# zhoubin-me/agent0

Hardware: AMD Instinct MI355X
Metric: env-frames/sec (learner FPS: transitions collected and saved to replay per second with the learner running, pre-frameskip) (higher is better)
Workload: dtype f32

## Files before the change

agent0_amd/csrc/conv1_wgrad.hip:

```cpp
#include "a0_internal.h"
#include "store_policy.h"
#include "update_tail.h"
typedef a0_st_wt a0_c1w_store;

#include <cstdint>

typedef __bf16 a0w_bf16x8 __attribute__((ext_vector_type(8)));
typedef uint32_t a0w_u32x4 __attribute__((ext_vector_type(4)));
typedef float a0w_acc4 __attribute__((ext_vector_type(4)));

constexpr int A0W_THREADS = 512;
constexpr int A0W_XP_ROW = 24, A0W_XP_PLANE = 21 * 24;
constexpr int A0W_XP_ELEMS = 64 * A0W_XP_PLANE;
constexpr int A0W_T_PITCH = 488, A0W_T_TERM = 32 * A0W_T_PITCH;
constexpr int A0W_GROUPS = 60;
constexpr int A0W_STEPS = 15;

struct a0_c1w_args {
    const uint8_t* frames; const int* slot; long long sample_stride; int chan_off;
    const float* d1;
    float* slabs;
    int B;
    a0_tail_prep prep;
};

A0_D uint32_t a0w_trunc(float f) { return __float_as_uint(f) >> 16; }
A0_D float a0w_up(uint32_t h) { return __uint_as_float(h << 16); }

__global__ __launch_bounds__(A0W_THREADS) void a0_conv1_wgrad_fused_kernel(a0_c1w_args P) {
    extern __shared__ __attribute__((aligned(16))) unsigned char smem[];
    uint16_t* Xp = (uint16_t*)smem;
    uint16_t* T = Xp + A0W_XP_ELEMS;
    const int tid = threadIdx.x, lane = tid & 63;
    const int wave = __builtin_amdgcn_readfirstlane(tid >> 6);
    const int q = lane >> 4, r16 = lane & 15;
    for (int i = tid; i < (A0W_XP_ELEMS + 3 * A0W_T_TERM) / 2; i += A0W_THREADS) ((uint32_t*)smem)[i] = 0u;
    int bbase[2], bshift[2];
#pragma unroll
    for (int t = 0; t < 2; ++t) {
        const int k = (2 * wave + t) * 16 + r16;
        const int c = k >> 6, kh = (k >> 3) & 7, kw = k & 7;
        const int plane = (c * 4 + (kh & 3)) * 4 + (kw & 3);
        bbase[t] = plane * A0W_XP_PLANE + (kh >> 2) * A0W_XP_ROW;
        bshift[t] = 2 * (kw >> 2);
    }
    a0w_acc4 acc[2][2];
#pragma unroll
    for (int i = 0; i < 2; ++i)
#pragma unroll
        for (int t = 0; t < 2; ++t) acc[i][t] = a0w_acc4{0.f, 0.f, 0.f, 0.f};
    float bsum = 0.f;
    __syncthreads();
    constexpr int NDW = 4 * 84 * 21, TR = (NDW + A0W_THREADS - 1) / A0W_THREADS;
    constexpr int GT = (A0W_GROUPS + A0W_THREADS / 32 - 1) / (A0W_THREADS / 32);
    uint32_t w[TR];
    float v[GT][8];
    auto load_raw = [&](int b) {
        const long long s = P.slot ? (long long)P.slot[b] : (long long)b;
        const uint32_t* src = (const uint32_t*)(P.frames + s * P.sample_stride + P.chan_off);
#pragma unroll
        for (int j = 0; j < TR; ++j) { const int i = tid + j * A0W_THREADS; w[j] = src[i < NDW ? i : NDW - 1]; }
        const float* g = P.d1 + (long long)b * 400 * 32 + (tid & 31);
#pragma unroll
        for (int t = 0; t < GT; ++t) {
            int G = (tid >> 5) + t * (A0W_THREADS / 32);
            G = G < A0W_GROUPS ? G : A0W_GROUPS - 1;
            const int oh = G / 3, ow0 = 8 * (G - 3 * oh);
#pragma unroll
            for (int j = 0; j < 8; ++j) { const int m = oh * 20 + ow0 + j; v[t][j] = g[(m < 400 ? m : 399) * 32]; }
        }
    };
    load_raw(blockIdx.x);
    for (int b = blockIdx.x; b < P.B; b += gridDim.x) {
#pragma unroll
        for (int j = 0; j < TR; ++j) {
            int i = tid + j * A0W_THREADS;
            i = i < NDW ? i : NDW - 1;
            const int c = i / (84 * 21), rem = i - c * (84 * 21), y = rem / 21, xc = rem - y * 21;
            uint16_t* d = Xp + ((c * 4 + (y & 3)) * 4) * A0W_XP_PLANE + (y >> 2) * A0W_XP_ROW + xc;
            d[0 * A0W_XP_PLANE] = (uint16_t)(__float_as_uint((float)(w[j] & 0xffu)) >> 16);
            d[1 * A0W_XP_PLANE] = (uint16_t)(__float_as_uint((float)((w[j] >> 8) & 0xffu)) >> 16);
            d[2 * A0W_XP_PLANE] = (uint16_t)(__float_as_uint((float)((w[j] >> 16) & 0xffu)) >> 16);
            d[3 * A0W_XP_PLANE] = (uint16_t)(__float_as_uint((float)(w[j] >> 24)) >> 16);
        }
        {
            const int n = tid & 31;
#pragma unroll
            for (int t = 0; t < GT; ++t) {
                const int G = (tid >> 5) + t * (A0W_THREADS / 32);
                if (G < A0W_GROUPS) {
                    const int oh = G / 3, ow0 = 8 * (G - 3 * oh);
                    uint32_t t0[4], t1[4], t2[4];
#pragma unroll
                    for (int j = 0; j < 8; j += 2) {
                        uint32_t h[2], m[2], l[2];
#pragma unroll
                        for (int e = 0; e < 2; ++e) {
                            const float x = (ow0 + j + e < 20) ? v[t][j + e] : 0.f;
                            bsum += x;
                            h[e] = a0w_trunc(x);
                            const float r1 = x - a0w_up(h[e]);
                            m[e] = a0w_trunc(r1);
                            l[e] = a0w_trunc(r1 - a0w_up(m[e]));
                        }
                        t0[j >> 1] = h[0] | (h[1] << 16); t1[j >> 1] = m[0] | (m[1] << 16); t2[j >> 1] = l[0] | (l[1] << 16);
                    }
                    uint16_t* d = T + n * A0W_T_PITCH + 8 * G;
                    *(uint4*)(d) = uint4{t0[0], t0[1], t0[2], t0[3]};
                    *(uint4*)(d + A0W_T_TERM) = uint4{t1[0], t1[1], t1[2], t1[3]};
                    *(uint4*)(d + 2 * A0W_T_TERM) = uint4{t2[0], t2[1], t2[2], t2[3]};
                }
            }
        }
        __syncthreads();
        if (b + (int)gridDim.x < P.B) load_raw(b + gridDim.x);
        {
            const uint16_t* ap = T + r16 * A0W_T_PITCH + 8 * q;
            const uint16_t* bp0 = Xp + bbase[0] + 8 * q;
            const uint16_t* bp1 = Xp + bbase[1] + 8 * q;
#pragma unroll 3
            for (int st = 0; st < A0W_STEPS; ++st) {
                a0w_u32x4 a[2][3], bf[2];
#pragma unroll
                for (int i = 0; i < 2; ++i)
#pragma unroll
                    for (int s3 = 0; s3 < 3; ++s3) {
                        const uint4 x = *(const uint4*)(ap + s3 * A0W_T_TERM + i * 16 * A0W_T_PITCH + 32 * st);
                        a[i][s3] = a0w_u32x4{x.x, x.y, x.z, x.w};
                    }
#pragma unroll
                for (int t = 0; t < 2; ++t) {
                    const uint16_t* bp = (t == 0 ? bp0 : bp1) + 32 * st;
                    const uint4 lo = *(const uint4*)bp;
                    const uint32_t hi = *(const uint32_t*)(bp + 8);
                    const int sh = bshift[t];
                    bf[t] = a0w_u32x4{__builtin_amdgcn_alignbyte(lo.y, lo.x, sh), __builtin_amdgcn_alignbyte(lo.z, lo.y, sh),
                                      __builtin_amdgcn_alignbyte(lo.w, lo.z, sh), __builtin_amdgcn_alignbyte(hi, lo.w, sh)};
                }
#pragma unroll
                for (int s3 = 0; s3 < 3; ++s3)
#pragma unroll
                    for (int i = 0; i < 2; ++i)
#pragma unroll
                        for (int t = 0; t < 2; ++t)
                            acc[i][t] = __builtin_amdgcn_mfma_f32_16x16x32_bf16(__builtin_bit_cast(a0w_bf16x8, a[i][s3]), __builtin_bit_cast(a0w_bf16x8, bf[t]), acc[i][t], 0, 0, 0);
            }
        }
        __syncthreads();
    }
    float* out = P.slabs + (long long)blockIdx.x * (32 * 256 + 32);
#pragma unroll
    for (int i = 0; i < 2; ++i)
#pragma unroll
        for (int t = 0; t < 2; ++t) {
            const int k = (2 * wave + t) * 16 + r16;
#pragma unroll
            for (int r = 0; r < 4; ++r) a0_store4<a0_c1w_store>(&out[(i * 16 + 4 * q + r) * 256 + k], __float_as_uint(acc[i][t][r] / 255.0f));
        }
    float* red = (float*)smem;
    red[tid] = bsum;
    __syncthreads();
    if (tid < 32) {
        float s = 0.f;
#pragma unroll
        for (int j = 0; j < A0W_THREADS / 32; ++j) s += red[j * 32 + tid];
        out[32 * 256 + tid] = s;
    }
    if (P.prep.state != nullptr && blockIdx.x == 0 && tid == 0) a0_tail_prep_run(P.prep);
}

int a0_conv1_wgrad_fused_launch(const a0_frames_arg* f, int C, int H, int W, int B, const float* d1, float* slabs, const a0_tail_prep* prep, hipStream_t st) {
    if (C != 4 || H != 84 || W != 84 || B < 1 || (f->sample_stride & 3) || (f->chan_off & 3) || (((uintptr_t)f->frames) & 3)) return 0;
    a0_c1w_args P;
    P.frames = f->frames; P.slot = f->slot; P.sample_stride = f->sample_stride; P.chan_off = f->chan_off;
    P.d1 = d1; P.slabs = slabs; P.B = B;
    P.prep = prep ? *prep : a0_tail_prep{nullptr, nullptr, 0.0, 0.0, 0.0, 0};
    const int grid = B < 256 ? B : 256;
    const size_t lds = (size_t)(A0W_XP_ELEMS + 3 * A0W_T_TERM) * 2;
    static bool configured = false;
    if (!configured) {
        A0_HIP_THROW(hipFuncSetAttribute((const void*)a0_conv1_wgrad_fused_kernel, hipFuncAttributeMaxDynamicSharedMemorySize, (int)lds));
        configured = true;
    }
    hipLaunchKernelGGL(a0_conv1_wgrad_fused_kernel, dim3(grid), dim3(A0W_THREADS), lds, st, P);
    A0_HIP_THROW(hipGetLastError());
    return grid;
}
```

agent0_amd/csrc/encoder_fused.hip:

```cpp
#include "a0_internal.h"
#include "net_tables.h"
#include "operands.h"
#include "store_policy.h"
#include "update_tail.h"

#include <cstdlib>
#include <type_traits>

typedef float a0_acc4 __attribute__((ext_vector_type(4)));

struct a0_fused_args {
    const uint8_t* frames; const int* slot; long long sample_stride; int chan_off;
    const float *wt1, *wt2, *wt3;
    const float *wx2, *wx3;
    const float *b1, *b2, *b3;
    float *act1, *act2, *act3;
    int B;
    int C, H, W, H1, W1, H2, W2, H3, W3;
    int off_act1, off_act2, off_end;
    int rp1, rp2;
};

A0_HD void a0_fused_set_wt(a0_fused_args& P, const float* wt, int C) {
    const a0_wt_layout T{C};
// ... 381 lines not shown
        *(a0_f4*)(glb + (unsigned)(m * N + n0)) = a0_f4{v[0], v[1], v[2], v[3]};
    }
};

struct a0_live_all {
    static constexpr bool all = true;
    static constexpr int steps = 2;
    static constexpr bool live(int, int) { return true; }
};
template <int ORD, int N, int WN, int MBT, int R, int LR, class LIVE = a0_live_all, class AFX, class EPI, class Between>
A0_D void a0_conv_stage_x9k(const AFX& af, int M, a0_wring9<N, WN, R, A0_FUSED_WAVES / WN>& ring, const EPI& epi, float* xch0, float* xch1, Between&& between) {
    constexpr int WK = A0_FUSED_WAVES / WN, HB0 = (MBT + 1) / 2, HB1 = MBT / 2;
    static_assert(WK == 2 && N == 16 * WN && HB1 >= 1 && EPI::TR && LR >= 1 && LR <= 16, "tile shape");
    const int tid = threadIdx.x, lane = tid & 63;
    const int wave = __builtin_amdgcn_readfirstlane(tid >> 6);
    const int wn = wave % WN, wk = wave / WN;
    const int q = lane >> 4, r16 = lane & 15;
    const int MB = (M + 15) >> 4, NSTW = LIVE::all ? ring.nst : LIVE::steps / WK;
    static_assert(LIVE::all || (LIVE::steps % (WK * R)) == 0, "own k steps: a multiple of the ring depth");
    auto live = [](int blk, int j) { return j < LIVE::steps / WK && (LIVE::live(blk, WK * j) || LIVE::live(blk, WK * j + 1)); };
    int rows[MBT];
#pragma unroll
    for (int i = 0; i < MBT; ++i) {
        const int m = i * 16 + r16;
        rows[i] = af.row(m < M ? m : 0) + 8 * q;
    }
    a0_acc4 acc[MBT];
#pragma unroll
    for (int i = 0; i < MBT; ++i) acc[i] = a0_acc4{0.f, 0.f, 0.f, 0.f};
    uint4 a[2][HB0][3];
    auto fetch = [&](int slot, int h, int off, int j) {
#pragma unroll
        for (int i = 0; i < HB0; ++i)
            if (h * HB0 + i < MBT) {
                if constexpr (!LIVE::all) { if (!live(h * HB0 + i, j)) continue; }
#pragma unroll
                for (int t = 0; t < 3; ++t) a[slot][i][t] = *(const uint4*)(af.planes + rows[h * HB0 + i] + off + t * AFX::term);
            }
    };
    fetch(0, 0, af.step_off(wk), 0);
    __builtin_amdgcn_s_waitcnt(0x0F70);
    if constexpr (!LIVE::all) asm volatile("" : "+v"(ring.p));
#pragma unroll LIVE::all ? 1 : LIVE::steps / (WK * R)
    for (int tb = 0; tb < NSTW; tb += R) {
#pragma unroll
        for (int u = 0; u < R; ++u) {
            const int st = wk + WK * (tb + u);
            const int off = af.step_off(st), offn = af.step_off(tb + u + 1 < NSTW ? st + WK : st);
#pragma unroll
            for (int h = 0; h < 2; ++h) {
                if (h == 0) fetch(1, 1, off, tb + u);
                else fetch(0, 0, offn, tb + u + 1);
                __builtin_amdgcn_sched_barrier(0);
#pragma unroll
                for (int ta = 0; ta < 3; ++ta)
#pragma unroll
                    for (int tw = 0; tw < 3; ++tw)
#pragma unroll
                        for (int i = 0; i < HB0; ++i) {
                            if (ta + tw > ORD || h * HB0 + i >= MBT) continue;
                            if constexpr (!LIVE::all) { if (!live(h * HB0 + i, tb + u)) continue; }
                            const a0_u32x4 av = {a[h][i][ta].x, a[h][i][ta].y, a[h][i][ta].z, a[h][i][ta].w};
                            const a0_u32x4 bv = {ring.v[u][0][tw].x, ring.v[u][0][tw].y, ring.v[u][0][tw].z, ring.v[u][0][tw].w};
                            acc[h * HB0 + i] = __builtin_amdgcn_mfma_f32_16x16x32_bf16(__builtin_bit_cast(a0_bf16x8, bv), __builtin_bit_cast(a0_bf16x8, av), acc[h * HB0 + i], 0, 0, 0);
                        }
                __builtin_amdgcn_sched_barrier(0);
            }
            ring.fill(u);
            __builtin_amdgcn_sched_barrier(0);
        }
    }
    between();
    a0_acc4* x0 = (a0_acc4*)xch0;
    a0_acc4* x1 = (a0_acc4*)xch1;
    constexpr int P1 = (HB1 - 1) * 64 + 4 * LR;
    const int last = q * LR + r16;
    const int n0 = wn * 16 + 4 * q;
    float pe[EPI::PER_ELEM ? HB0 : 1][4];
    auto send = [&](auto mine) {
        constexpr int H = decltype(mine)::value;
        if constexpr (EPI::PER_ELEM) {
#pragma unroll
            for (int i = 0; i < (H == 0 ? HB0 : HB1); ++i) {
                const int m = (H * HB0 + i) * 16 + r16;
                const a0_f4 v = epi.pre_elem4(m < M ? m : M - 1, n0);
                pe[i][0] = v.x; pe[i][1] = v.y; pe[i][2] = v.z; pe[i][3] = v.w;
            }
        }
        if constexpr (H == 1) {
#pragma unroll
            for (int i = 0; i < HB0; ++i) x0[(wn * HB0 + i) * 64 + lane] = acc[i];
        } else {
#pragma unroll
            for (int i = 0; i < HB1; ++i) {
                if (i < HB1 - 1) x1[wn * P1 + i * 64 + lane] = acc[HB0 + i];
                else if (r16 < LR) x1[wn * P1 + (HB1 - 1) * 64 + last] = acc[HB0 + i];
            }
        }
    };
    auto recv = [&](auto mine) {
        constexpr int H = decltype(mine)::value;
#pragma unroll
        for (int i = 0; i < (H == 0 ? HB0 : HB1); ++i) {
            const int mb = H * HB0 + i;
            const int m = mb * 16 + r16;
            if constexpr (H == 0) acc[mb] += x0[(wn * HB0 + i) * 64 + lane];
            else {
                if (i < HB1 - 1) acc[mb] += x1[wn * P1 + i * 64 + lane];
                else if (r16 < LR) acc[mb] += x1[wn * P1 + (HB1 - 1) * 64 + last];
            }
            if (mb < MB && m < M) epi.emit_n4(m, n0, acc[mb], EPI::PER_ELEM ? pe[EPI::PER_ELEM ? i : 0] : nullptr);
        }
    };
    if (wk == 0) send(std::integral_constant<int, 0>{});
    else send(std::integral_constant<int, 1>{});
    __syncthreads();
    if (wk == 0) recv(std::integral_constant<int, 0>{});
    else recv(std::integral_constant<int, 1>{});
    __syncthreads();
}
constexpr int A0_P1X = 40, A0_P2X = 80;
constexpr int A0_RP1X = 20 * A0_P1X + 8;
constexpr int A0_RP2X = 9 * A0_P2X + 96;

constexpr int A0_R1 = 4, A0_R2 = 4, A0_R3 = 6;

template <int MBW1, int MBW2, int MBW3, int WC, bool X9, bool LOOP = false, int ORD = 4>
__global__ __launch_bounds__(A0_FUSED_THREADS) void a0_encoder_fused_kernel(a0_fused_args P);

constexpr int A0_X9_BIAS_OFF = 2 * 4 * 84 * 84 + 3 * 20 * A0_RP1X * 2;
constexpr int A0_RK2 = 2, A0_RK3 = 3;
constexpr int A0_X9_XCH0 = 3 * 9 * A0_RP2X * 2;
constexpr int A0_X9_XCH1 = A0_X9_BIAS_OFF + 160 * 4;
static_assert(A0_X9_XCH0 + 4 * 3 * 1024 <= 2 * 4 * 84 * 84, "conv2 exchange region 0 fits into the image");
constexpr int A0_X9_LDS_BYTES = A0_X9_XCH1 + 4 * (2 * 64 + 4) * 16;
static_assert(A0_X9_LDS_BYTES <= 160 * 1024, "LDS");
static_assert(A0_FUSED_WAVES == 8, "N-stationary stages: four waves along N, two along K");
typedef a0_wring9<64, 4, A0_RK2, 2> a0_ring2_t;
typedef a0_wring9<64, 4, A0_RK3, 2> a0_ring3_t;
template <int ORD, bool LOOP>
A0_D void a0_x9_conv23(const a0_fused_args& P, int b, unsigned char* smem, float* bias_lds, a0_wring1<A0_R1>& ring1, a0_ring2_t& ring2, a0_ring3_t& ring3) {
    const int obs_bytes = P.C * P.H * P.W;
    const int M2 = P.H2 * P.W2, M3 = P.H3 * P.W3;
    uint16_t* a1p = (uint16_t*)(smem + 2 * obs_bytes);
    constexpr int term1 = 20 * A0_RP1X, term2 = 9 * A0_RP2X;
    uint16_t* a2p = (uint16_t*)smem;
    typedef EpiFwdX<9, A0_P2X, A0_RP2X, term2> E2X;
    const AF2X<term1> f2{a1p, A0_RP1X, P.W2, A0_P1X};
    const E2X e2{bias_lds + 32, a2p, P.act2 ? P.act2 + (long long)b * M2 * 64 : nullptr, 64};
    const AF3X<term2> f3{a2p, A0_RP2X, P.W3, A0_P2X};
    const EpiFwdT e3{bias_lds + 96, P.act3 + (long long)b * M3 * 64, 64};
    a0_conv_stage_x9k<ORD, 64, 4, 6, A0_RK2, 1>(f2, M2, ring2, e2, (float*)(smem + A0_X9_XCH0), (float*)(smem + A0_X9_XCH1), [&] { ring3.prologue(); });
    a0_conv_stage_x9k<ORD, 64, 4, 4, A0_RK3, 16>(f3, M3, ring3, e3, (float*)a1p, (float*)a1p + 4 * 2 * 256, [&] { if (LOOP) ring1.prologue(); });
}

A0_D void a0_bytes16_to_img(uint16_t* img, int idx16, const uint4& v) {
    const uint32_t w[4] = {v.x, v.y, v.z, v.w};
    uint32_t o[8];
#pragma unroll
    for (int k = 0; k < 4; ++k) {
        const uint32_t f0 = __float_as_uint((float)(w[k] & 0xffu)), f1 = __float_as_uint((float)((w[k] >> 8) & 0xffu));
        const uint32_t f2 = __float_as_uint((float)((w[k] >> 16) & 0xffu)), f3 = __float_as_uint((float)(w[k] >> 24));
        o[2 * k] = __builtin_amdgcn_perm(f1, f0, 0x07060302u);
        o[2 * k + 1] = __builtin_amdgcn_perm(f3, f2, 0x07060302u);
    }
    ((uint4*)img)[2 * idx16] = uint4{o[0], o[1], o[2], o[3]};
    ((uint4*)img)[2 * idx16 + 1] = uint4{o[4], o[5], o[6], o[7]};
}

template <int ORD, bool LOOP>
A0_D void a0_encoder_fused_x9_body(const a0_fused_args& P, int bid, int nblk) {
    extern __shared__ __attribute__((aligned(16))) unsigned char smem[];
    uint16_t* img = (uint16_t*)smem;
    const int obs_bytes = P.C * P.H * P.W;
    const int M1 = P.H1 * P.W1;
    uint16_t* a1p = (uint16_t*)(smem + 2 * obs_bytes);
    constexpr int term1 = 20 * A0_RP1X;
    typedef EpiFwdX<20, A0_P1X, A0_RP1X, term1> E1X;
    a0_wring1<A0_R1> ring1;
    a0_ring2_t ring2;
    a0_ring3_t ring3;
    ring1.init(P.wt1, P.C);
    ring2.init(P.wx2, 512);
    ring3.init(P.wx3, 576);
    ring1.prologue();
    constexpr int MBW1X = (25 + A0_WMG1 - 1) / A0_WMG1;
    a0_pre<32, 2, MBW1X, E1X> pre1;
    float* bias_lds = (float*)(smem + A0_X9_BIAS_OFF);
    if (threadIdx.x < 160) bias_lds[threadIdx.x] = threadIdx.x < 32 ? P.b1[threadIdx.x] : threadIdx.x < 96 ? P.b2[threadIdx.x - 32] : P.b3[threadIdx.x - 96];
    for (int b = bid; b < P.B; b += nblk) {
        const long long s = P.slot ? (long long)P.slot[b] : (long long)b;
        const uint4* src = (const uint4*)(P.frames + s * P.sample_stride + P.chan_off);
        constexpr int TRIPS = 4;
        const int n16 = obs_bytes >> 4;
        for (int i0 = threadIdx.x; i0 < n16; i0 += TRIPS * A0_FUSED_THREADS) {
            uint4 v[TRIPS];
#pragma unroll
            for (int j = 0; j < TRIPS; ++j) {
                const int i = i0 + j * A0_FUSED_THREADS;
                v[j] = src[i < n16 ? i : n16 - 1];
            }
#pragma unroll
            for (int j = 0; j < TRIPS; ++j) {
                const int i = i0 + j * A0_FUSED_THREADS;
                a0_bytes16_to_img(img, i < n16 ? i : n16 - 1, v[j]);
            }
        }
        __syncthreads();
        const E1X e1{bias_lds, a1p, P.act1 ? P.act1 + (long long)b * M1 * 32 : nullptr, 32};
        const int wmg1 = __builtin_amdgcn_readfirstlane(threadIdx.x >> 6) / 2;
        if (MBW1X > 1 && wmg1 + (MBW1X - 1) * A0_WMG1 >= ((M1 + 15) >> 4))
            a0_conv1_stage<(MBW1X > 1 ? MBW1X - 1 : 1), A0_R1, 84>(img, P.H * P.W, P.W, P.W1, M1, ring1, e1, pre1, [&] { ring2.prologue(); });
        else
            a0_conv1_stage<MBW1X, A0_R1, 84>(img, P.H * P.W, P.W, P.W1, M1, ring1, e1, pre1, [&] { ring2.prologue(); });
        a0_x9_conv23<ORD, LOOP>(P, b, smem, bias_lds, ring1, ring2, ring3);
        if constexpr (!LOOP) break;
    }
}

#include "actor_tail.h"
typedef a0_st_nt a0_step_row_store;
struct a0_step_enc_args { const float *wt, *b1, *b2, *b3; float* act3; };
template <int ORD>
__global__ __launch_bounds__(A0_FUSED_THREADS) void a0_actor_dist_step_enc_kernel(a0_dtenv_args Q, a0_step_enc_args N) {
    __shared__ int s_chase_cell;
    extern __shared__ __attribute__((aligned(16))) unsigned char smem[];
    unsigned long long v_wt = (unsigned long long)N.wt, v_b1 = (unsigned long long)N.b1, v_b2 = (unsigned long long)N.b2, v_b3 = (unsigned long long)N.b3,
                       v_a3 = (unsigned long long)N.act3, v_obs = (unsigned long long)Q.obs_out;
    A0_TO_VGPR(v_wt); A0_TO_VGPR(v_b1); A0_TO_VGPR(v_b2); A0_TO_VGPR(v_b3); A0_TO_VGPR(v_a3); A0_TO_VGPR(v_obs);
    int v_E = Q.E;
    A0_TO_VGPR(v_E);
    a0_actor_dist_tail_env_body(Q, (float*)smem, &s_chase_cell);
    __syncthreads();
    auto uni = [](unsigned long long v) {
        return ((unsigned long long)(unsigned)__builtin_amdgcn_readfirstlane((int)(v >> 32)) << 32) | (unsigned long long)(unsigned)__builtin_amdgcn_readfirstlane((int)(v & 0xffffffffull));
    };
    const float* wt = (const float*)uni(v_wt);
    a0_fused_args P;
    P.frames = (const uint8_t*)uni(v_obs); P.slot = nullptr; P.sample_stride = 4 * 84 * 84; P.chan_off = 0;
    a0_fused_set_wt(P, wt, 4);
    P.b1 = (const float*)uni(v_b1); P.b2 = (const float*)uni(v_b2); P.b3 = (const float*)uni(v_b3);
    P.act1 = nullptr; P.act2 = nullptr; P.act3 = (float*)uni(v_a3); P.B = __builtin_amdgcn_readfirstlane(v_E);
    P.C = 4; P.H = 84; P.W = 84; P.H1 = 20; P.W1 = 20; P.H2 = 9; P.W2 = 9; P.H3 = 7; P.W3 = 7;
    P.off_act1 = 0; P.off_act2 = 0; P.off_end = 0; P.rp1 = 0; P.rp2 = 0;
    a0_encoder_fused_x9_body<ORD, false>(P, (int)blockIdx.x, (int)gridDim.x);
}

template <int MBW, class EPI, class Mid, class Between>
A0_D void a0_conv1_stage_split(const uint16_t* img, a0_wring1<A0_R1>& ring, const EPI& epi, bool first_before_mid, Mid&& mid, Between&& between) {
    static_assert(A0_R1 == 4 && EPI::TR, "ring of four steps, transposed accumulators");
    constexpr int HW = 84 * 84, W = 84, W1 = 20, M = 400, MB = 25;
    const int tid = threadIdx.x, lane = tid & 63;
    const int wave = __builtin_amdgcn_readfirstlane(tid >> 6);
    const int wn = wave % 2, wmg = wave / 2;
    const int q = lane >> 4, r16 = lane & 15;
    int rows[MBW];
#pragma unroll
    for (int i = 0; i < MBW; ++i) {
        int m = (wmg + i * A0_WMG1) * 16 + r16;
        m = m < M ? m : 0;
        const int oh = m / W1, ow = m - oh * W1;
        rows[i] = (4 * oh + q) * W + 4 * ow;
    }
    a0_acc4 acc[MBW];
#pragma unroll
    for (int i = 0; i < MBW; ++i) acc[i] = a0_acc4{0.f, 0.f, 0.f, 0.f};
    uint2 a[2][MBW][2];
    auto fetch = [&](int slot, int off) {
#pragma unroll
        for (int i = 0; i < MBW; ++i) {
            a[slot][i][0] = *(const uint2*)(img + rows[i] + off);
            a[slot][i][1] = *(const uint2*)(img + rows[i] + off + 4);
        }
    };
    auto off_of = [&](int st) { return (st >> 1) * HW + (st & 1) * 4 * W; };
    auto step = [&](auto UC, int off_next) {
        constexpr int u = decltype(UC)::value;
        fetch((u + 1) & 1, off_next);
        __builtin_amdgcn_sched_barrier(0);
#pragma unroll
        for (int s3 = 0; s3 < 3; ++s3)
#pragma unroll
            for (int i = 0; i < MBW; ++i) {
                const a0_u32x4 av = {a[u & 1][i][0].x, a[u & 1][i][0].y, a[u & 1][i][1].x, a[u & 1][i][1].y};
                const a0_u32x4 bv = {ring.v[u][s3].x, ring.v[u][s3].y, ring.v[u][s3].z, ring.v[u][s3].w};
                acc[i] = __builtin_amdgcn_mfma_f32_16x16x32_bf16(__builtin_bit_cast(a0_bf16x8, bv), __builtin_bit_cast(a0_bf16x8, av), acc[i], 0, 0, 0);
            }
        __builtin_amdgcn_sched_barrier(0);
        ring.fill(u);
        __builtin_amdgcn_sched_barrier(0);
    };
    typedef std::integral_constant<int, 0> U0; typedef std::integral_constant<int, 1> U1; typedef std::integral_constant<int, 2> U2; typedef std::integral_constant<int, 3> U3;
    auto steps05 = [&] {
        fetch(0, off_of(0));
        __builtin_amdgcn_s_waitcnt(0x0F70);
        step(U0{}, off_of(1)); step(U1{}, off_of(2)); step(U2{}, off_of(3)); step(U3{}, off_of(4));
        step(U0{}, off_of(5)); step(U1{}, off_of(5));
    };
    if (first_before_mid) steps05();
    mid();
    if (!first_before_mid) steps05();
    fetch(0, off_of(6));
    __builtin_amdgcn_s_waitcnt(0x0F70);
    step(U2{}, off_of(7)); step(U3{}, off_of(7));
    between();
#pragma unroll
    for (int i = 0; i < MBW; ++i) {
        const int mb = wmg + i * A0_WMG1;
        if (mb < MB) {
            const int m = mb * 16 + r16;
            if (m < M) epi.emit_n4(m, wn * 16 + 4 * q, acc[i], nullptr);
        }
    }
    __syncthreads();
}

struct TailScalar {
    typedef a0_qenv_args Args;
    static A0_D void run(const a0_qenv_args& Q, uint32_t e, uint32_t g, long long steps, unsigned long long off_a, unsigned long long off_u, float eps, long long slot, const a0_u4& x,
                         bool chase, int lane, float* w2s , float* raw, int* s_chase_cell_p) {
// ... 615 lines not shown
```

agent0_amd/csrc/operands.h:

```cpp
#pragma once
#include "a0_defs.h"
#include "store_policy.h"

enum { A0_KC = 0, A0_XC = 1 };

struct a0_frames_src {
    const uint8_t* frames;
    const int* slot;
    a0_geom g;
    int chan_off;
    const a0_i4* ktab;
    int aligned4;
};

A0_HD uint32_t a0_u8x4_load(const uint8_t* p, int aligned4) {
    if (aligned4) return *(const uint32_t*)p;
    return (uint32_t)p[0] | ((uint32_t)p[1] << 8) | ((uint32_t)p[2] << 16) | ((uint32_t)p[3] << 24);
}

A0_HD float a0_div255(float x) {
    const float r = 1.0f / 255.0f;
    const float q0 = x * r;
#if defined(__HIPCC__)
    const float e = __builtin_fmaf(-q0, 255.0f, x);
    return __builtin_fmaf(e, r, q0);
#else
    const float e = __builtin_fmaf(-q0, 255.0f, x);
    return __builtin_fmaf(e, r, q0);
#endif
}

A0_HD a0_f4 a0_u8x4_to_f4(uint32_t w, bool valid) {
    if (!valid) w = 0;
    a0_f4 v;
    v.x = a0_div255((float)(w & 255u));
    v.y = a0_div255((float)((w >> 8) & 255u));
    v.z = a0_div255((float)((w >> 16) & 255u));
    v.w = a0_div255((float)(w >> 24));
    return v;
}

A0_HD const uint8_t* a0_frames_row(const a0_frames_src& P, int m) {
    int b = a0_udiv(m, P.g.HWout, P.g.hw_magic);
    int rem = m - b * P.g.HWout;
    int oh = a0_udiv(rem, P.g.Wout, P.g.w_magic);
    int ow = rem - oh * P.g.Wout;
    long long s = P.slot ? (long long)P.slot[b] : (long long)b;
    return P.frames + s * P.g.sample_stride + P.chan_off + (long long)(oh * P.g.stride) * P.g.Win + ow * P.g.stride;
}

struct OpFramesKC {
    static constexpr int MODE = A0_KC;
    typedef a0_frames_src Params;
    struct Row { const uint8_t* p; bool ok; };
    struct KInfo { int off; bool ok; };
    A0_HD static Row row(const Params& P, int m, int M) {
        Row r; r.ok = m < M; r.p = a0_frames_row(P, r.ok ? m : 0); return r;
    }
    A0_HD static KInfo kinfo(const Params& P, int k, int Kend) {
        KInfo ki; ki.ok = k < Kend; ki.off = P.ktab[ki.ok ? (k >> 2) : 0].x; return ki;
    }
    typedef uint32_t Raw;
    A0_HD static Raw load(const Params& P, const Row& r, const KInfo& ki, bool& ok) {
        ok = r.ok && ki.ok;
        return a0_u8x4_load(r.p + ki.off, P.aligned4);
    }
    A0_HD static a0_f4 finish(Raw w, bool ok) { return a0_u8x4_to_f4(w, ok); }
};

struct OpFramesXC {
    static constexpr int MODE = A0_XC;
    typedef a0_frames_src Params;
    struct XInfo { int off; bool ok; };
    A0_HD static XInfo xinfo(const Params& P, int x, int X) {
        XInfo xi; xi.ok = x < X; xi.off = P.ktab[xi.ok ? (x >> 2) : 0].x; return xi;
    }
    typedef uint32_t Raw;
    A0_HD static Raw load(const Params& P, int m, int Mend, const XInfo& xi, bool& ok) {
        ok = xi.ok && m < Mend;
        return a0_u8x4_load(a0_frames_row(P, ok ? m : 0) + xi.off, P.aligned4);
    }
    A0_HD static a0_f4 finish(Raw w, bool ok) { return a0_u8x4_to_f4(w, ok); }
};

struct a0_act_src {
    const float* x;
    a0_geom g;
    const a0_i4* ktab;
};

struct a0_act_row { long long base; int h0, w0; bool ok; };

A0_HD a0_act_row a0_act_rowdesc(const a0_act_src& P, int m, bool ok) {
    a0_act_row r;
    if (!ok) m = 0;
    int b = a0_udiv(m, P.g.HWout, P.g.hw_magic);
    int rem = m - b * P.g.HWout;
    int oh = a0_udiv(rem, P.g.Wout, P.g.w_magic);
    int ow = rem - oh * P.g.Wout;
    r.h0 = oh * P.g.stride - P.g.pad;
    r.w0 = ow * P.g.stride - P.g.pad;
    r.base = (long long)b * P.g.sample_stride + ((long long)r.h0 * P.g.Win + r.w0) * P.g.C;
    r.ok = ok;
    return r;
}

A0_HD a0_f4 a0_act_fetch(const a0_act_src& P, const a0_act_row& r, const a0_i4& t, bool kok, bool& ok) {
    const int h = r.h0 + t.y, w = r.w0 + t.z;
    ok = r.ok && kok && (unsigned)h < (unsigned)P.g.Hin && (unsigned)w < (unsigned)P.g.Win;
    return *(const a0_f4*)(P.x + (ok ? r.base + t.x : 0));
}

A0_HD a0_f4 a0_f4_select(a0_f4 v, bool ok) { if (!ok) v = a0_zero4(); return v; }

struct OpActKC {
    static constexpr int MODE = A0_KC;
    typedef a0_act_src Params;
    typedef a0_act_row Row;
    struct KInfo { a0_i4 t; bool ok; };
    A0_HD static Row row(const Params& P, int m, int M) { return a0_act_rowdesc(P, m, m < M); }
    A0_HD static KInfo kinfo(const Params& P, int k, int Kend) {
        KInfo ki; ki.ok = k < Kend; ki.t = P.ktab[ki.ok ? (k >> 2) : 0]; return ki;
    }
    typedef a0_f4 Raw;
    A0_HD static Raw load(const Params& P, const Row& r, const KInfo& ki, bool& ok) { return a0_act_fetch(P, r, ki.t, ki.ok, ok); }
    A0_HD static a0_f4 finish(Raw v, bool ok) { return a0_f4_select(v, ok); }
};

struct OpActXC {
    static constexpr int MODE = A0_XC;
    typedef a0_act_src Params;
    struct XInfo { a0_i4 t; bool ok; };
    A0_HD static XInfo xinfo(const Params& P, int x, int X) {
        XInfo xi; xi.ok = x < X; xi.t = P.ktab[xi.ok ? (x >> 2) : 0]; return xi;
    }
    typedef a0_f4 Raw;
    A0_HD static Raw load(const Params& P, int m, int Mend, const XInfo& xi, bool& ok) {
        return a0_act_fetch(P, a0_act_rowdesc(P, m, m < Mend), xi.t, xi.ok, ok);
    }
    A0_HD static a0_f4 finish(Raw v, bool ok) { return a0_f4_select(v, ok); }
};

struct a0_mat_src { const float* x; int ld; };

struct OpMatKC {
    static constexpr int MODE = A0_KC;
    typedef a0_mat_src Params;
    struct Row { const float* p; bool ok; };
    struct KInfo { int k; bool ok; };
    A0_HD static Row row(const Params& P, int r, int R) { Row o; o.ok = r < R; o.p = P.x + (o.ok ? (long long)r * P.ld : 0); return o; }
    A0_HD static KInfo kinfo(const Params&, int k, int Kend) { KInfo ki; ki.ok = k < Kend; ki.k = ki.ok ? k : 0; return ki; }
    typedef a0_f4 Raw;
    A0_HD static Raw load(const Params&, const Row& r, const KInfo& ki, bool& ok) {
        ok = r.ok && ki.ok;
        return *(const a0_f4*)(r.p + ki.k);
    }
    A0_HD static a0_f4 finish(Raw v, bool ok) { return a0_f4_select(v, ok); }
};

struct OpMatXC {
    static constexpr int MODE = A0_XC;
    typedef a0_mat_src Params;
    struct XInfo { int x; bool ok; };
    A0_HD static XInfo xinfo(const Params&, int x, int X) { XInfo xi; xi.ok = x < X; xi.x = xi.ok ? x : 0; return xi; }
    typedef a0_f4 Raw;
    A0_HD static Raw load(const Params& P, int k, int Kend, const XInfo& xi, bool& ok) {
        ok = xi.ok && k < Kend;
        return *(const a0_f4*)(P.x + (ok ? (long long)k * P.ld : 0) + xi.x);
    }
    A0_HD static a0_f4 finish(Raw v, bool ok) { return a0_f4_select(v, ok); }
};

struct a0_wtab_src { const float* w; const int* wtab; };

struct OpWtabXC {
    static constexpr int MODE = A0_XC;
    typedef a0_wtab_src Params;
    struct XInfo { int x; bool ok; };
    A0_HD static XInfo xinfo(const Params&, int x, int X) { XInfo xi; xi.ok = x < X; xi.x = xi.ok ? x : 0; return xi; }
    typedef a0_f4 Raw;
    A0_HD static Raw load(const Params& P, int k, int Kend, const XInfo& xi, bool& ok) {
        ok = xi.ok && k < Kend;
        return *(const a0_f4*)(P.w + P.wtab[ok ? k : 0] + xi.x);
    }
    A0_HD static a0_f4 finish(Raw v, bool ok) { return a0_f4_select(v, ok); }
};

struct EpiBiasAct {
    static constexpr bool ROWSUM_A = false;
    struct Params { float* out; const float* bias; int ld; int relu; };
    A0_HD static void store(const Params& P, int x, int y, float v, int) {
        v += P.bias[y];
        if (P.relu) v = (v < 0.f) ? 0.f : v;
// ... 59 lines not shown
```

Measured before the change: 2.567 million.

## Restructure conv1 wgrad LDS layout using transposed LDS reads and plain image

Rewrites the conv1 weight-gradient kernel to stage the frame as a row-major bf16 image (reusing the shared bytes-to-image helper) and the d1 gradient in a swizzled 64-byte-row layout. MFMA fragments are then fetched with ds_read_tr16_b64 transposed LDS reads, replacing the stride-4 phase-plane layout and the alignbyte shuffles. Global loads become 16-byte vector loads, the per-iteration LDS zeroing shrinks to padding only, and the bias sum is rebuilt from the fragments already loaded. In exchange it relies on the MI355X-specific transpose-read instruction and tighter padding and swizzle invariants, which carry correctness risk.

```diff
diff --git a/agent0_amd/csrc/conv1_wgrad.hip b/agent0_amd/csrc/conv1_wgrad.hip
--- a/agent0_amd/csrc/conv1_wgrad.hip
+++ b/agent0_amd/csrc/conv1_wgrad.hip
@@ -1,4 +1,5 @@
 #include "a0_internal.h"
+#include "operands.h"
 #include "store_policy.h"
 #include "update_tail.h"
 typedef a0_st_wt a0_c1w_store;
@@ -6,15 +7,23 @@
 #include <cstdint>
 
 typedef __bf16 a0w_bf16x8 __attribute__((ext_vector_type(8)));
+typedef short a0w_s16x4 __attribute__((ext_vector_type(4)));
+typedef uint32_t a0w_u32x2 __attribute__((ext_vector_type(2)));
 typedef uint32_t a0w_u32x4 __attribute__((ext_vector_type(4)));
 typedef float a0w_acc4 __attribute__((ext_vector_type(4)));
+typedef uint32_t a0w_u32x4_a4 __attribute__((ext_vector_type(4), aligned(4)));
+typedef float a0w_f32x4_a4 __attribute__((ext_vector_type(4), aligned(4)));
 
 constexpr int A0W_THREADS = 512;
-constexpr int A0W_XP_ROW = 24, A0W_XP_PLANE = 21 * 24;
-constexpr int A0W_XP_ELEMS = 64 * A0W_XP_PLANE;
-constexpr int A0W_T_PITCH = 488, A0W_T_TERM = 32 * A0W_T_PITCH;
-constexpr int A0W_GROUPS = 60;
+constexpr int A0W_ROW = 64;
+constexpr int A0W_T_TERM = 20 * 24 * A0W_ROW;
+constexpr int A0W_IMG_PITCH = 84 * 2, A0W_IMG_CHAN = 84 * A0W_IMG_PITCH;
+constexpr int A0W_IMG_BYTES = 4 * A0W_IMG_CHAN;
+constexpr int A0W_IMG_TAIL = 32;
+constexpr int A0W_LDS_BYTES = 3 * A0W_T_TERM + A0W_IMG_BYTES + A0W_IMG_TAIL;
 constexpr int A0W_STEPS = 15;
+static_assert((3 * A0W_T_TERM) % 256 == 0 && A0W_IMG_BYTES % 16 == 0, "the image starts on a bank row; 16-byte stores reach its tail");
+static_assert(3 * A0W_IMG_CHAN + (4 * 19 + 7) * A0W_IMG_PITCH + 2 * (4 * 23 + 4) + 8 == A0W_IMG_BYTES + A0W_IMG_TAIL, "the last transposed read ends with the tail");
 
 struct a0_c1w_args {
     const uint8_t* frames; const int* slot; long long sample_stride; int chan_off;
@@ -24,25 +33,78 @@
     a0_tail_prep prep;
 };
 
-A0_D uint32_t a0w_trunc(float f) { return __float_as_uint(f) >> 16; }
-A0_D float a0w_up(uint32_t h) { return __uint_as_float(h << 16); }
+A0_D void a0w_split4(const a0_f4& v, a0w_u32x2& hi, a0w_u32x2& mid, a0w_u32x2& lo) {
+    const float x[4] = {v.x, v.y, v.z, v.w};
+    uint32_t h[4], m[4], l[4];
+#pragma unroll
+    for (int e = 0; e < 4; ++e) {
+        h[e] = __float_as_uint(x[e]);
+        const float r1 = x[e] - __uint_as_float(h[e] & 0xffff0000u);
+        m[e] = __float_as_uint(r1);
+        l[e] = __float_as_uint(r1 - __uint_as_float(m[e] & 0xffff0000u));
+    }
+    hi.x = __builtin_amdgcn_perm(h[1], h[0], 0x07060302u);  hi.y = __builtin_amdgcn_perm(h[3], h[2], 0x07060302u);
+    mid.x = __builtin_amdgcn_perm(m[1], m[0], 0x07060302u); mid.y = __builtin_amdgcn_perm(m[3], m[2], 0x07060302u);
+    lo.x = __builtin_amdgcn_perm(l[1], l[0], 0x07060302u);  lo.y = __builtin_amdgcn_perm(l[3], l[2], 0x07060302u);
+}
+
+A0_D a0w_u32x4 a0w_frag(const unsigned char* p0, const unsigned char* p1) {
+    typedef __attribute__((address_space(3))) a0w_s16x4 lds_s16x4;
+    const a0w_s16x4 k03 = __builtin_amdgcn_ds_read_tr16_b64_v4i16((lds_s16x4*)p0);
+    const a0w_s16x4 k47 = __builtin_amdgcn_ds_read_tr16_b64_v4i16((lds_s16x4*)p1);
+    const a0w_u32x2 a = __builtin_bit_cast(a0w_u32x2, k03), b = __builtin_bit_cast(a0w_u32x2, k47);
+    return a0w_u32x4{a.x, a.y, b.x, b.y};
+}
 
 __global__ __launch_bounds__(A0W_THREADS) void a0_conv1_wgrad_fused_kernel(a0_c1w_args P) {
     extern __shared__ __attribute__((aligned(16))) unsigned char smem[];
-    uint16_t* Xp = (uint16_t*)smem;
-    uint16_t* T = Xp + A0W_XP_ELEMS;
+    unsigned char* const T = smem;
+    unsigned char* const img = smem + 3 * A0W_T_TERM;
     const int tid = threadIdx.x, lane = tid & 63;
     const int wave = __builtin_amdgcn_readfirstlane(tid >> 6);
     const int q = lane >> 4, r16 = lane & 15;
-    for (int i = tid; i < (A0W_XP_ELEMS + 3 * A0W_T_TERM) / 2; i += A0W_THREADS) ((uint32_t*)smem)[i] = 0u;
-    int bbase[2], bshift[2];
+    constexpr int N16 = 4 * 84 * 84 / 16, TR = (N16 + A0W_THREADS - 1) / A0W_THREADS;
+    constexpr int NF4 = 400 * 8, TD = (NF4 + A0W_THREADS - 1) / A0W_THREADS;
+    uint4 w[TR];
+    a0_f4 v[TD];
+    auto load_raw = [&](int b) {
+        const long long s = P.slot ? (long long)P.slot[b] : (long long)b;
+        const uint8_t* src = P.frames + s * P.sample_stride + P.chan_off;
+        const float* g = P.d1 + (long long)b * 400 * 32;
+#pragma unroll
+        for (int j = 0; j < TR; ++j) {
+            const int i = tid + j * A0W_THREADS;
+            const a0w_u32x4_a4 x = ((const a0w_u32x4_a4*)src)[i < N16 ? i : N16 - 1];
+            w[j] = uint4{x[0], x[1], x[2], x[3]};
+        }
+#pragma unroll
+        for (int j = 0; j < TD; ++j) {
+            const int i = tid + j * A0W_THREADS;
+            const a0w_f32x4_a4 x = ((const a0w_f32x4_a4*)g)[i < NF4 ? i : NF4 - 1];
+            v[j].x = x[0]; v[j].y = x[1]; v[j].z = x[2]; v[j].w = x[3];
+        }
+    };
+    load_raw(blockIdx.x);
+    for (int i = tid; i < 3 * 20 * 16 + A0W_IMG_TAIL / 16; i += A0W_THREADS) {
+        const int term = i / 320, rem = i - term * 320;
+        unsigned char* d = i < 960 ? T + term * A0W_T_TERM + ((rem >> 4) * 24 + 20) * A0W_ROW + (rem & 15) * 16 : img + A0W_IMG_BYTES + (i - 960) * 16;
+        *(uint4*)d = uint4{0u, 0u, 0u, 0u};
+    }
+    int doff[TD];
+#pragma unroll
+    for (int j = 0; j < TD; ++j) {
+        int i = tid + j * A0W_THREADS;
+        i = i < NF4 ? i : NF4 - 1;
+        const int pos = i >> 3, m = pos + 4 * (pos / 20);
+        doff[j] = m * A0W_ROW + ((8 * (i & 7)) ^ (32 * ((m >> 3) & 1)));
+    }
+    const int fr = r16 >> 2, fp = r16 & 3;
+    const int aoff = (8 * q + fr) * A0W_ROW + ((8 * fp) ^ (32 * (q & 1)));
+    int bbase[2];
 #pragma unroll
     for (int t = 0; t < 2; ++t) {
-        const int k = (2 * wave + t) * 16 + r16;
-        const int c = k >> 6, kh = (k >> 3) & 7, kw = k & 7;
-        const int plane = (c * 4 + (kh & 3)) * 4 + (kw & 3);
-        bbase[t] = plane * A0W_XP_PLANE + (kh >> 2) * A0W_XP_ROW;
-        bshift[t] = 2 * (kw >> 2);
+        const int tb = 2 * wave + t, c = tb >> 2, kh0 = 2 * (tb & 3);
+        bbase[t] = c * A0W_IMG_CHAN + (kh0 + (fp >> 1)) * A0W_IMG_PITCH + 8 * (fp & 1) + 8 * fr;
     }
     a0w_acc4 acc[2][2];
 #pragma unroll
@@ -50,100 +112,49 @@
 #pragma unroll
         for (int t = 0; t < 2; ++t) acc[i][t] = a0w_acc4{0.f, 0.f, 0.f, 0.f};
     float bsum = 0.f;
-    __syncthreads();
-    constexpr int NDW = 4 * 84 * 21, TR = (NDW + A0W_THREADS - 1) / A0W_THREADS;
-    constexpr int GT = (A0W_GROUPS + A0W_THREADS / 32 - 1) / (A0W_THREADS / 32);
-    uint32_t w[TR];
-    float v[GT][8];
-    auto load_raw = [&](int b) {
-        const long long s = P.slot ? (long long)P.slot[b] : (long long)b;
-        const uint32_t* src = (const uint32_t*)(P.frames + s * P.sample_stride + P.chan_off);
-#pragma unroll
-        for (int j = 0; j < TR; ++j) { const int i = tid + j * A0W_THREADS; w[j] = src[i < NDW ? i : NDW - 1]; }
-        const float* g = P.d1 + (long long)b * 400 * 32 + (tid & 31);
-#pragma unroll
-        for (int t = 0; t < GT; ++t) {
-            int G = (tid >> 5) + t * (A0W_THREADS / 32);
-            G = G < A0W_GROUPS ? G : A0W_GROUPS - 1;
-            const int oh = G / 3, ow0 = 8 * (G - 3 * oh);
-#pragma unroll
-            for (int j = 0; j < 8; ++j) { const int m = oh * 20 + ow0 + j; v[t][j] = g[(m < 400 ? m : 399) * 32]; }
-        }
-    };
-    load_raw(blockIdx.x);
     for (int b = blockIdx.x; b < P.B; b += gridDim.x) {
 #pragma unroll
-        for (int j = 0; j < TR; ++j) {
-            int i = tid + j * A0W_THREADS;
-            i = i < NDW ? i : NDW - 1;
-            const int c = i / (84 * 21), rem = i - c * (84 * 21), y = rem / 21, xc = rem - y * 21;
-            uint16_t* d = Xp + ((c * 4 + (y & 3)) * 4) * A0W_XP_PLANE + (y >> 2) * A0W_XP_ROW + xc;
-            d[0 * A0W_XP_PLANE] = (uint16_t)(__float_as_uint((float)(w[j] & 0xffu)) >> 16);
-            d[1 * A0W_XP_PLANE] = (uint16_t)(__float_as_uint((float)((w[j] >> 8) & 0xffu)) >> 16);
-            d[2 * A0W_XP_PLANE] = (uint16_t)(__float_as_uint((float)((w[j] >> 16) & 0xffu)) >> 16);
-            d[3 * A0W_XP_PLANE] = (uint16_t)(__float_as_uint((float)(w[j] >> 24)) >> 16);
-        }
-        {
-            const int n = tid & 31;
+        for (int j = 0; j < TR; ++j) { const int i = tid + j * A0W_THREADS; a0_bytes16_to_img((uint16_t*)img, i < N16 ? i : N16 - 1, w[j]); }
 #pragma unroll
-            for (int t = 0; t < GT; ++t) {
-                const int G = (tid >> 5) + t * (A0W_THREADS / 32);
-                if (G < A0W_GROUPS) {
-                    const int oh = G / 3, ow0 = 8 * (G - 3 * oh);
-                    uint32_t t0[4], t1[4], t2[4];
-#pragma unroll
-                    for (int j = 0; j < 8; j += 2) {
-                        uint32_t h[2], m[2], l[2];
-#pragma unroll
-                        for (int e = 0; e < 2; ++e) {
-                            const float x = (ow0 + j + e < 20) ? v[t][j + e] : 0.f;
-                            bsum += x;
-                            h[e] = a0w_trunc(x);
-                            const float r1 = x - a0w_up(h[e]);
-                            m[e] = a0w_trunc(r1);
-                            l[e] = a0w_trunc(r1 - a0w_up(m[e]));
-                        }
-                        t0[j >> 1] = h[0] | (h[1] << 16); t1[j >> 1] = m[0] | (m[1] << 16); t2[j >> 1] = l[0] | (l[1] << 16);
-                    }
-                    uint16_t* d = T + n * A0W_T_PITCH + 8 * G;
-                    *(uint4*)(d) = uint4{t0[0], t0[1], t0[2], t0[3]};
-                    *(uint4*)(d + A0W_T_TERM) = uint4{t1[0], t1[1], t1[2], t1[3]};
-                    *(uint4*)(d + 2 * A0W_T_TERM) = uint4{t2[0], t2[1], t2[2], t2[3]};
-                }
-            }
+        for (int j = 0; j < TD; ++j) {
+            a0w_u32x2 hi, mid, lo;
+            a0w_split4(v[j], hi, mid, lo);
+            unsigned char* d = T + doff[j];
+            *(a0w_u32x2*)d = hi; *(a0w_u32x2*)(d + A0W_T_TERM) = mid; *(a0w_u32x2*)(d + 2 * A0W_T_TERM) = lo;
         }
         __syncthreads();
         if (b + (int)gridDim.x < P.B) load_raw(b + gridDim.x);
-        {
-            const uint16_t* ap = T + r16 * A0W_T_PITCH + 8 * q;
-            const uint16_t* bp0 = Xp + bbase[0] + 8 * q;
-            const uint16_t* bp1 = Xp + bbase[1] + 8 * q;
 #pragma unroll 3
-            for (int st = 0; st < A0W_STEPS; ++st) {
-                a0w_u32x4 a[2][3], bf[2];
+        for (int st = 0; st < A0W_STEPS; ++st) {
+            a0w_u32x4 a[2][3], bf[2];
+#pragma unroll
+            for (int i = 0; i < 2; ++i)
+#pragma unroll
+                for (int s3 = 0; s3 < 3; ++s3) {
+                    const unsigned char* x = T + (aoff ^ (32 * i)) + s3 * A0W_T_TERM + 32 * A0W_ROW * st;
+                    a[i][s3] = a0w_frag(x, x + 4 * A0W_ROW);
+                }
+            {
+                const unsigned G = 4u * st + q, oh = G / 3u;
+                const unsigned char* bp = img + oh * (4 * A0W_IMG_PITCH) + (G - 3u * oh) * 64;
+#pragma unroll
+                for (int t = 0; t < 2; ++t) bf[t] = a0w_frag(bp + bbase[t], bp + bbase[t] + 32);
+            }
+#pragma unroll
+            for (int s3 = 0; s3 < 3; ++s3)
 #pragma unroll
                 for (int i = 0; i < 2; ++i)
 #pragma unroll
-                    for (int s3 = 0; s3 < 3; ++s3) {
-                        const uint4 x = *(const uint4*)(ap + s3 * A0W_T_TERM + i * 16 * A0W_T_PITCH + 32 * st);
-                        a[i][s3] = a0w_u32x4{x.x, x.y, x.z, x.w};
-                    }
+                    for (int t = 0; t < 2; ++t)
+                        acc[i][t] = __builtin_amdgcn_mfma_f32_16x16x32_bf16(__builtin_bit_cast(a0w_bf16x8, a[i][s3]), __builtin_bit_cast(a0w_bf16x8, bf[t]), acc[i][t], 0, 0, 0);
+            if (((st ^ wave) & 3) == 0) {
+                const bool up = wave >= 4;
 #pragma unroll
-                for (int t = 0; t < 2; ++t) {
-                    const uint16_t* bp = (t == 0 ? bp0 : bp1) + 32 * st;
-                    const uint4 lo = *(const uint4*)bp;
-                    const uint32_t hi = *(const uint32_t*)(bp + 8);
-                    const int sh = bshift[t];
-                    bf[t] = a0w_u32x4{__builtin_amdgcn_alignbyte(lo.y, lo.x, sh), __builtin_amdgcn_alignbyte(lo.z, lo.y, sh),
-                                      __builtin_amdgcn_alignbyte(lo.w, lo.z, sh), __builtin_amdgcn_alignbyte(hi, lo.w, sh)};
+                for (int e = 0; e < 4; ++e) {
+                    const uint32_t h = up ? a[1][0][e] : a[0][0][e], m = up ? a[1][1][e] : a[0][1][e], l = up ? a[1][2][e] : a[0][2][e];
+                    bsum += (__uint_as_float(h << 16) + __uint_as_float(m << 16)) + __uint_as_float(l << 16);
+                    bsum += (__uint_as_float(h & 0xffff0000u) + __uint_as_float(m & 0xffff0000u)) + __uint_as_float(l & 0xffff0000u);
                 }
-#pragma unroll
-                for (int s3 = 0; s3 < 3; ++s3)
-#pragma unroll
-                    for (int i = 0; i < 2; ++i)
-#pragma unroll
-                        for (int t = 0; t < 2; ++t)
-                            acc[i][t] = __builtin_amdgcn_mfma_f32_16x16x32_bf16(__builtin_bit_cast(a0w_bf16x8, a[i][s3]), __builtin_bit_cast(a0w_bf16x8, bf[t]), acc[i][t], 0, 0, 0);
             }
         }
         __syncthreads();
@@ -158,7 +169,7 @@
             for (int r = 0; r < 4; ++r) a0_store4<a0_c1w_store>(&out[(i * 16 + 4 * q + r) * 256 + k], __float_as_uint(acc[i][t][r] / 255.0f));
         }
     float* red = (float*)smem;
-    red[tid] = bsum;
+    red[(4 * (wave & 3) + q) * 32 + 16 * (wave >> 2) + r16] = bsum;
     __syncthreads();
     if (tid < 32) {
         float s = 0.f;
@@ -176,7 +187,7 @@
     P.d1 = d1; P.slabs = slabs; P.B = B;
     P.prep = prep ? *prep : a0_tail_prep{nullptr, nullptr, 0.0, 0.0, 0.0, 0};
     const int grid = B < 256 ? B : 256;
-    const size_t lds = (size_t)(A0W_XP_ELEMS + 3 * A0W_T_TERM) * 2;
+    const size_t lds = (size_t)A0W_LDS_BYTES;
     static bool configured = false;
     if (!configured) {
         A0_HIP_THROW(hipFuncSetAttribute((const void*)a0_conv1_wgrad_fused_kernel, hipFuncAttributeMaxDynamicSharedMemorySize, (int)lds));
diff --git a/agent0_amd/csrc/encoder_fused.hip b/agent0_amd/csrc/encoder_fused.hip
--- a/agent0_amd/csrc/encoder_fused.hip
+++ b/agent0_amd/csrc/encoder_fused.hip
@@ -557,20 +557,6 @@
     const EpiFwdT e3{bias_lds + 96, P.act3 + (long long)b * M3 * 64, 64};
     a0_conv_stage_x9k<ORD, 64, 4, 6, A0_RK2, 1>(f2, M2, ring2, e2, (float*)(smem + A0_X9_XCH0), (float*)(smem + A0_X9_XCH1), [&] { ring3.prologue(); });
     a0_conv_stage_x9k<ORD, 64, 4, 4, A0_RK3, 16>(f3, M3, ring3, e3, (float*)a1p, (float*)a1p + 4 * 2 * 256, [&] { if (LOOP) ring1.prologue(); });
-}
-
-A0_D void a0_bytes16_to_img(uint16_t* img, int idx16, const uint4& v) {
-    const uint32_t w[4] = {v.x, v.y, v.z, v.w};
-    uint32_t o[8];
-#pragma unroll
-    for (int k = 0; k < 4; ++k) {
-        const uint32_t f0 = __float_as_uint((float)(w[k] & 0xffu)), f1 = __float_as_uint((float)((w[k] >> 8) & 0xffu));
-        const uint32_t f2 = __float_as_uint((float)((w[k] >> 16) & 0xffu)), f3 = __float_as_uint((float)(w[k] >> 24));
-        o[2 * k] = __builtin_amdgcn_perm(f1, f0, 0x07060302u);
-        o[2 * k + 1] = __builtin_amdgcn_perm(f3, f2, 0x07060302u);
-    }
-    ((uint4*)img)[2 * idx16] = uint4{o[0], o[1], o[2], o[3]};
-    ((uint4*)img)[2 * idx16 + 1] = uint4{o[4], o[5], o[6], o[7]};
 }
 
 template <int ORD, bool LOOP>
diff --git a/agent0_amd/csrc/operands.h b/agent0_amd/csrc/operands.h
--- a/agent0_amd/csrc/operands.h
+++ b/agent0_amd/csrc/operands.h
@@ -39,6 +39,22 @@
     v.w = a0_div255((float)(w >> 24));
     return v;
 }
+
+#if defined(__HIPCC__)
+A0_D void a0_bytes16_to_img(uint16_t* img, int idx16, const uint4& v) {
+    const uint32_t w[4] = {v.x, v.y, v.z, v.w};
+    uint32_t o[8];
+#pragma unroll
+    for (int k = 0; k < 4; ++k) {
+        const uint32_t f0 = __float_as_uint((float)(w[k] & 0xffu)), f1 = __float_as_uint((float)((w[k] >> 8) & 0xffu));
+        const uint32_t f2 = __float_as_uint((float)((w[k] >> 16) & 0xffu)), f3 = __float_as_uint((float)(w[k] >> 24));
+        o[2 * k] = __builtin_amdgcn_perm(f1, f0, 0x07060302u);
+        o[2 * k + 1] = __builtin_amdgcn_perm(f3, f2, 0x07060302u);
+    }
+    ((uint4*)img)[2 * idx16] = uint4{o[0], o[1], o[2], o[3]};
+    ((uint4*)img)[2 * idx16 + 1] = uint4{o[4], o[5], o[6], o[7]};
+}
+#endif
 
 A0_HD const uint8_t* a0_frames_row(const a0_frames_src& P, int m) {
     int b = a0_udiv(m, P.g.HWout, P.g.hw_magic);
```

New measurement: 2.581 million (median of 6 runs). Within noise of the previous version (+0.5%).
